# osmocom/osmo-trx

Measured on AMD Instinct MI355X. Metric: Mbursts/s detect+demod (156.25 sym, 4 SPS), higher is better.
Workload: dtype f32

## Files before the change

osmo_trx_amd/csrc/trx_kernel_nb.hip:

```cpp
#include "trx_k4_common.h"
#include "trx_nb_asm.inc"

#define NB_D_LEN    160
#define NB_CZ_LEN   (TRX_CZ_PAD + TRX_CORR_NARROW + TRX_CZ_PAD)
#define NB_SLICE    (K4_XS + NB_D_LEN + NB_CZ_LEN)
#define NB_COMP_ROWS (TRX_DELAY_FILTS + 1)
#define NB_TABLES_FLOATS (TRX_SINCV_LDS + 16 * WAVE + NB_COMP_ROWS * 36 + 16 + 8 * 8 + 5 * WAVE + 5 * WAVE + 2 * 8 * 16)
#define NB_TABLES_BYTES (NB_TABLES_FLOATS * 4)
#define NB_WPB 16
#define NB_POOL_RING 64
#define NB_POOL_UNSET (-1)
#define NB_POOL_END (-2)
#define NB_NO_BURST 0xffffffffu
#define NB_LDS_TAIL (16 + 4 * NB_POOL_RING)
#define NB_LDS_BYTES (NB_TABLES_BYTES + NB_WPB * NB_SLICE * 8 + NB_LDS_TAIL)
#define NB_MAX_TOA 32



typedef float v3f __attribute__((ext_vector_type(3)));
typedef int v4i __attribute__((ext_vector_type(4)));

template <typename T>
__device__ __forceinline__ unsigned lds_addr(const T *p)
// ... 42 lines not shown
		wa4f[((u >> 2) * WAVE + l) * 4 + (u & 3)] = (q < TRX_SINCV_LEN) ? tab->sincv[q] : 0.0f;
	}
	for (int i = threadIdx.x; i < NB_COMP_ROWS * 36; i += blockDim.x) {
		const int f = i / 36, j = i % 36;
		comp[i] = (j >= TRX_FUSED_SH) ? tab->comp_filt[f][j - TRX_FUSED_SH] : 0.0f;
	}
	if (threadIdx.x < 16)
		gdec[threadIdx.x] = tab->dec_taps[threadIdx.x];
	if (threadIdx.x < 128)
		lseq[threadIdx.x] = make_float2(tab->seq[TRX_SEQ_TSC0 + (threadIdx.x >> 4)].taps[threadIdx.x & 15].re,
						tab->seq[TRX_SEQ_TSC0 + (threadIdx.x >> 4)].taps[threadIdx.x & 15].im);
	if (threadIdx.x < 64)
		lhdr[threadIdx.x] = reinterpret_cast<const float *>(&tab->seq[TRX_SEQ_TSC0 + (threadIdx.x >> 3)].gain)[threadIdx.x & 7];
	if (threadIdx.x < WAVE) {
		const PeakConst pc0 = peak_const(threadIdx.x);
		pkcl[0 * WAVE + threadIdx.x] = pc0.flA;
		pkcl[1 * WAVE + threadIdx.x] = pc0.loA;
		pkcl[2 * WAVE + threadIdx.x] = pc0.hiA;
		pkcl[3 * WAVE + threadIdx.x] = pc0.offB;
		pkcl[4 * WAVE + threadIdx.x] = pc0.ratio_off;
		lcn[0 * WAVE + threadIdx.x] = pc0.ratio_off * 8;
		lcn[1 * WAVE + threadIdx.x] = (pc0.flA - 8) * 8;
		lcn[2 * WAVE + threadIdx.x] = pc0.offB;
		const int l = threadIdx.x, e = (-l) & 3;
		const bool sp = l >= 52 && l < 60;
		lcn[3 * WAVE + l] = 8 * (sp ? (l < 56 ? e : e - 2) : (l < 48 ? 4 + 3 * l : 148));
		lcn[4 * WAVE + l] = sp ? (e + (l >= 56 ? 4 : 0)) * K4_NTP * 4 : -1;
	}
	for (int i = lane0; i < NB_SLICE; i += WAVE)
		wbase[i] = make_float2(0.0f, 0.0f);
	if (threadIdx.x == 0) {
		wg_next[0] = NB_WPB;
		wg_next[1] = 0;
	}
	if (threadIdx.x < NB_POOL_RING)
		pool_g[threadIdx.x] = NB_POOL_UNSET;
	__syncthreads();

	const float fs_db = 6.02059991f * __log2f(full_scale);
	const float thr2 = thresh * thresh;
	const float gc0 = thr2 * 1.0001e-5f;
	int t5pk = 0;
	bool t5_ok = true;
	for (int t = 0; t < 8; t++) {
		const int v = (int)(lhdr[8 * t + 5] * 512.0f);
		t5_ok = t5_ok && v >= -8 && v <= 7 && (float)v == lhdr[8 * t + 5] * 512.0f;
		t5pk |= (v & 15) << (4 * t);
	}
	t5pk = uni(t5pk);
	const unsigned long long e8_addr = reinterpret_cast<unsigned long long>(&tab->edge8[0][0][0]);
// ... 161 lines not shown
			float ar = x0.x * ct0, ai = x0.y * ct0;
			ar = fmaf(x1.x, ct1, ar); ai = fmaf(x1.y, ct1, ai);
			ar = fmaf(x2.x, ct2, ar); ai = fmaf(x2.y, ct2, ai);
			const float sr = row_sum(ar), si = row_sum(ai);
			if (lt == 0 && lact)
				dec[li] = cmul(make_float2(sr, si), scale);
		}
		if (hi_tab) {
			const int s0 = 4 * hi_i - 24 - w + lt;
			const c32 *pp = P + ((s0 & 3) * PH_A + PH_M0 + (s0 >> 2));
			const c32 x0 = lds_c32(pp), x1 = lds_c32(pp + 4), x2 = lds_c32(pp + 8);
			float ar = x0.x * ch0, ai = x0.y * ch0;
			ar = fmaf(x1.x, ch1, ar); ai = fmaf(x1.y, ch1, ai);
			ar = fmaf(x2.x, ch2, ar); ai = fmaf(x2.y, ch2, ai);
			const float sr = row_sum(ar), si = row_sum(ai);
			if (lt == 0 && hact && hi_i < 156)
				dec[hi_i] = cmul(make_float2(sr, si), scale);
		}
		wave_sync();
		auto pick = [&](int i) {
			const float d = reinterpret_cast<const float *>(dec + i)[i & 1];
			return __builtin_amdgcn_fmed3f(fmaf((i & 2) ? -0.5f : 0.5f, d, 0.5f), 0.0f, 1.0f);
		};
		const int i0 = (lane < 48) ? 4 + 3 * lane : ((-lane) & 3);
		o.x = pick(i0);
		o.y = pick(lane < 48 ? i0 + 1 : 0);
		o.z = pick(lane < 48 ? i0 + 2 : 0);
		wave_sync();
		return true;
	};

	DIAG_DECL;
	unsigned j_next = 0, b_next = NB_NO_BURST;
	for (unsigned b = b_first; b != NB_NO_BURST; b = b_next) {
		int lane;
		asm volatile("v_mbcnt_lo_u32_b32 %0, -1, 0\n\tv_mbcnt_hi_u32_b32 %0, -1, %0" : "=v"(lane));
		const int ticket = claim_issue(wg_next);
		const unsigned prm0 = (unsigned)uni((int)pre_prm);
		const unsigned max_toa = prm0 >> 16;
		const int tsc = (prm0 >> 8) & 0xff;
		bool leave = ((prm0 & 0xf8ffu) != (unsigned)TRXHIP_TSC) || (max_toa > NB_MAX_TOA) || !t5_ok;

		c32 *const pload = P + (lane & 3) * PH_A + PH_M0 + (lane >> 2);
		float amax = 0.0f, epart = 0.0f;
#ifdef TRX_DIAG
		DIAG_MARK(12);
		asm volatile("s_waitcnt vmcnt(0)" ::: "memory");
		DIAG_MARK(13);
#endif
		if (!leave) {
#pragma unroll
			for (int r = 0; r < NLD; r++) {
				const int i = r * WAVE + lane;
				if (r < NLD - 1 || i < 625) {
					const c32 v = make_float2((float)(int16_t)(pre_i[r] & 0xffffu), (float)(int16_t)(pre_i[r] >> 16));
					pload[16 * r] = v;
					asm("v_max3_f32 %0, %0, |%1|, |%2|" : "+v"(amax) : "v"(v.x), "v"(v.y));
					if (r < 5)
						epart = fmaf(v.x, v.x, fmaf(v.y, v.y, epart));
				}
			}
		} else {
#pragma unroll
			for (int r = 0; r < NLD; r++)
				asm volatile("" :: "v"(pre_i[r]));
		}
		DIAG_MARK(14);
		if (pend_any) {
			float *const so = soft + (size_t)pend_b * 148;
			int *const rp = reinterpret_cast<int *>(results + pend_b);
			const float oe = o.x;
			asm volatile("s_bfm_b64 exec, 48, 0\n\t"
				     "global_store_dwordx3 %0, %1, %2 offset:16\n\t"
				     "s_bfm_b64 exec, 4, 52\n\t"
				     "global_store_dword %3, %4, %2\n\t"
				     "s_mov_b64 exec, %8\n\t"
				     "global_store_dword %5, %6, %7\n\t"
				     "s_mov_b64 exec, -1\n\t"
				     "s_nop 0"
				     :: "v"(lane * 12), "v"(o), "s"(so), "v"(((-lane) & 3) * 4), "v"(oe), "v"(lane * 4), "v"(recw), "s"(rp),
				        "s"(pend_rec ? 0xffull : 0ull)
				     : "memory");
		}
		pend_any = false;
		DIAG_MARK(16);
		j_next = (unsigned)(leave ? claim_take(ticket) : claim_take_behind<5>(ticket));
		b_next = burst_of(j_next);
		if (pooled && (j_next & 15u) == 0u && j_next + 16u >= items)
			pool_draw(j_next, b_next == NB_NO_BURST && j_next >= items, lane);
		DIAG_MARK(17);
		if (b_next != NB_NO_BURST)
			prefetch(b_next, lane);
		DIAG_MARK(15);

		int clip = 0;
		if (!leave) {
			clip = __ballot(amax > TRX_CLIP_THRESH) != 0ull;

			const int len = 16 + (int)max_toa;
			__builtin_assume(len >= 16 && len <= 16 + NB_MAX_TOA);
			const unsigned vd_addr = lds_addr(D) + 8u * (unsigned)lane, vcz_addr = lds_addr(cz) + 8u * (unsigned)lane;
			unsigned long long bad;
			float dr, di;
// ... 127 lines not shown
			}
		}
		if (leave) {
			if (lane == 0) {
				reinterpret_cast<uint8_t *>(redo + TRX_REDO_HDR)[b] = 1;
				if (!left_any)
					__hip_atomic_store(redo, 1u, __ATOMIC_RELAXED, __HIP_MEMORY_SCOPE_AGENT);
			}
			left_any = true;
			continue;
		}
		pend_b = b;
		pend_any = true;
		if (q_n == WAVE)
			flush_records(lane);
		DIAG_MARK(11);
	}
	if (pend_any) {
		int lane;
		asm volatile("v_mbcnt_lo_u32_b32 %0, -1, 0\n\tv_mbcnt_hi_u32_b32 %0, -1, %0" : "=v"(lane));
		float *const so = soft + (size_t)pend_b * 148;
		int *const rp = reinterpret_cast<int *>(results + pend_b);
		const float oe = o.x;
		asm volatile("s_bfm_b64 exec, 48, 0\n\t"
			     "global_store_dwordx3 %0, %1, %2 offset:16\n\t"
			     "s_bfm_b64 exec, 4, 52\n\t"
			     "global_store_dword %3, %4, %2\n\t"
			     "s_mov_b64 exec, %8\n\t"
			     "global_store_dword %5, %6, %7\n\t"
			     "s_mov_b64 exec, -1\n\t"
			     "s_nop 0"
			     :: "v"(lane * 12), "v"(o), "s"(so), "v"(((-lane) & 3) * 4), "v"(oe), "v"(lane * 4), "v"(recw), "s"(rp),
			        "s"(pend_rec ? 0xffull : 0ull)
			     : "memory");
	}
	{
		int lane;
		asm volatile("v_mbcnt_lo_u32_b32 %0, -1, 0\n\tv_mbcnt_hi_u32_b32 %0, -1, %0" : "=v"(lane));
		flush_records(lane);
	}
	DIAG_FLUSH();
	if (pooled) {
		__syncthreads();
		int tid0;
		asm volatile("v_mbcnt_lo_u32_b32 %0, -1, 0\n\tv_mbcnt_hi_u32_b32 %0, -1, %0" : "=v"(tid0));
		if (tid0 == 0 && atomicAdd(wg_next + 1, 1) == 0) {
			const unsigned d = __hip_atomic_fetch_add(pool_ctr + 1, 1u, __ATOMIC_ACQ_REL, __HIP_MEMORY_SCOPE_AGENT);
			if (d == gridDim.x - 1u) {
				__hip_atomic_store(pool_ctr, 0u, __ATOMIC_RELAXED, __HIP_MEMORY_SCOPE_AGENT);
				__hip_atomic_store(pool_ctr + 1, 0u, __ATOMIC_RELEASE, __HIP_MEMORY_SCOPE_AGENT);
			}
		}
	}
}
```

osmo_trx_amd/csrc/trx_nb_asm.inc:

```
#define NB_ASM_GDEC_OFF 29968
#define NB_ASM_LSEQ_OFF 32848
#define NB_ASM_DEC_MAX_NACT 60
#define NB_ASM_CORR_LANE0 19
#define NB_ASM_CORR_MAX_LEN 45
#define NB_ASM_CLOBBERS "v64", "v65", "v66", "v67", "v68", "v69", "v70", "v71", "v72", "v73", "v74", "v75", "v76", "v77", "v78", "v79", "v80", "v81", "v82", "v83", "v84", "v85", "v86", "v87", "v88", "v89", "v90", "v91", "v92", "v93", "v94", "v95", "v96", "v97", "v98", "v99", "v100", "v101", "v102", "v103", "v104", "v105", "v106", "v107", "v108", "v109", "v110", "v111", "v112", "v113", "v114", "v115", "v116", "v117", "v118", "v119", "v120", "v121", "v122", "v123", "v124", "v125", "v126", "v127", "s87", "s88", "s89", "s90", "s91", "s92", "s93", "s94", "s95", "s96", "s97", "s98", "s99", "vcc", "scc", "memory"
#define NB_ASM_DEC \
	"s_cmp_gt_u32 %[nact], 60\n\t" \
	"s_cbranch_scc1 .Lnb_dec_wide\n\t" \
	"s_sub_u32 s88, 60, %[nact]\n\t" \
	"s_lshr_b64 exec, -1, s88\n\t" \
	"ds_read_b128 v[120:123], %[zero] offset:29968\n\t" \
	"ds_read_b128 v[124:127], %[zero] offset:29984\n\t" \
	"ds_read_b64 v[98:99], %[pd] offset:1440\n\t" \
	"ds_read_b64 v[100:101], %[pd] offset:2880\n\t" \
	"ds_read_b64 v[102:103], %[pd] offset:4320\n\t" \
	"ds_read_b64 v[96:97], %[pd] offset:0\n\t" \
	"s_waitcnt lgkmcnt(3)\n\t" \
	"v_pk_mul_f32 v[64:65], v[98:99], v[120:121] op_sel:[0,0] op_sel_hi:[1,0]\n\t" \
	"s_waitcnt lgkmcnt(2)\n\t" \
	"v_pk_mul_f32 v[66:67], v[100:101], v[120:121] op_sel:[0,1] op_sel_hi:[1,1]\n\t" \
	"s_waitcnt lgkmcnt(1)\n\t" \
	"v_pk_mul_f32 v[68:69], v[102:103], v[122:123] op_sel:[0,0] op_sel_hi:[1,0]\n\t" \
	"v_pk_add_f32 v[104:105], v[64:65], v[66:67]\n\t" \
	"s_waitcnt lgkmcnt(0)\n\t" \
// ... 1448 lines not shown
	"s_add_u32 s95, s95, %[cb]\n\t" \
	"v_readlane_b32 %[ssum], v81, 0\n\t" \
	"s_mov_b64 exec, -1\n\t" \
	"s_sub_u32 s96, 0, s88\n\t" \
	"s_cmp_gt_u32 s96, 36\n\t" \
	"s_cbranch_scc1 .Lnb_tl_wait_end\n\t" \
	"s_mov_b32 %[ok], 1\n\t" \
	"v_add_u32_e32 v112, s94, %[kic]\n\t" \
	"s_add_u32 s96, s92, 1\n\t" \
	"s_lshr_b32 s96, s96, 2\n\t" \
	"s_mul_i32 s96, s96, -5752\n\t" \
	"s_add_u32 s96, s96, 1440\n\t" \
	"v_add_u32_e32 v113, s96, v112\n\t" \
	"s_add_u32 s96, s92, 2\n\t" \
	"s_lshr_b32 s96, s96, 2\n\t" \
	"s_mul_i32 s96, s96, -5752\n\t" \
	"s_add_u32 s96, s96, 2880\n\t" \
	"v_add_u32_e32 v114, s96, v112\n\t" \
	"s_add_u32 s96, s92, 3\n\t" \
	"s_lshr_b32 s96, s96, 2\n\t" \
	"s_mul_i32 s96, s96, -5752\n\t" \
	"s_add_u32 s96, s96, 4320\n\t" \
	"v_add_u32_e32 v115, s96, v112\n\t" \
	"s_mov_b32 exec_hi, 0x0ff0ffff\n\t" \
	"ds_read_b64 v[72:73], v112 offset:96\n\t" \
	"ds_read_b64 v[74:75], v113 offset:96\n\t" \
	"ds_read_b64 v[76:77], v114 offset:96\n\t" \
	"ds_read_b64 v[78:79], v115 offset:96\n\t" \
	"ds_read_b64 v[80:81], v112 offset:104\n\t" \
	"ds_read_b64 v[82:83], v113 offset:104\n\t" \
	"ds_read_b64 v[84:85], v114 offset:104\n\t" \
	"ds_read_b64 v[86:87], v115 offset:104\n\t" \
	"ds_read_b64 v[88:89], v112 offset:112\n\t" \
	"ds_read_b64 v[90:91], v113 offset:112\n\t" \
	"ds_read_b64 v[92:93], v114 offset:112\n\t" \
	"ds_read_b64 v[94:95], v115 offset:112\n\t" \
	"v_add_u32_e32 v116, %[db], %[l16]\n\t" \
	"v_cmp_lt_i32_e32 vcc, -1, %[ktp]\n\t" \
	"v_add_u32_e32 v117, %[db], %[ktp]\n\t" \
	"v_mov_b32_e32 v118, s95\n\t" \
	"v_mov_b64_e32 v[64:65], 0\n\t" \
	"v_mov_b64_e32 v[66:67], 0\n\t" \
	"v_mov_b64_e32 v[68:69], 0\n\t" \
	"v_cndmask_b32_e32 v117, v118, v117, vcc\n\t" \
	"s_waitcnt vmcnt(0)\n\t" \
	"ds_write_b128 v116, v[120:123]\n\t" \
	"ds_read_b128 v[104:107], v117\n\t" \
	"ds_read_b128 v[108:111], v117 offset:16\n\t" \
	"ds_read_b64 v[96:97], v112 offset:120\n\t" \
	"ds_read_b64 v[98:99], v113 offset:120\n\t" \
	"ds_read_b64 v[100:101], v114 offset:120\n\t" \
	"ds_read_b64 v[102:103], v115 offset:120\n\t" \
	"s_waitcnt lgkmcnt(5)\n\t" \
	"v_pk_fma_f32 v[64:65], v[72:73], v[104:105], v[64:65] op_sel:[0,0,0] op_sel_hi:[1,0,1]\n\t" \
	"v_pk_fma_f32 v[66:67], v[80:81], v[104:105], v[66:67] op_sel:[0,0,0] op_sel_hi:[1,0,1]\n\t" \
	"v_pk_fma_f32 v[68:69], v[88:89], v[104:105], v[68:69] op_sel:[0,0,0] op_sel_hi:[1,0,1]\n\t" \
	"v_pk_fma_f32 v[64:65], v[74:75], v[104:105], v[64:65] op_sel:[0,1,0] op_sel_hi:[1,1,1]\n\t" \
	"v_pk_fma_f32 v[66:67], v[82:83], v[104:105], v[66:67] op_sel:[0,1,0] op_sel_hi:[1,1,1]\n\t" \
	"v_pk_fma_f32 v[68:69], v[90:91], v[104:105], v[68:69] op_sel:[0,1,0] op_sel_hi:[1,1,1]\n\t" \
	"v_pk_fma_f32 v[64:65], v[76:77], v[106:107], v[64:65] op_sel:[0,0,0] op_sel_hi:[1,0,1]\n\t" \
	"v_pk_fma_f32 v[66:67], v[84:85], v[106:107], v[66:67] op_sel:[0,0,0] op_sel_hi:[1,0,1]\n\t" \
	"v_pk_fma_f32 v[68:69], v[92:93], v[106:107], v[68:69] op_sel:[0,0,0] op_sel_hi:[1,0,1]\n\t" \
	"v_pk_fma_f32 v[64:65], v[78:79], v[106:107], v[64:65] op_sel:[0,1,0] op_sel_hi:[1,1,1]\n\t" \
	"v_pk_fma_f32 v[66:67], v[86:87], v[106:107], v[66:67] op_sel:[0,1,0] op_sel_hi:[1,1,1]\n\t" \
	"v_pk_fma_f32 v[68:69], v[94:95], v[106:107], v[68:69] op_sel:[0,1,0] op_sel_hi:[1,1,1]\n\t" \
	"ds_read_b128 v[104:107], v117 offset:32\n\t" \
	"ds_read_b64 v[72:73], v112 offset:128\n\t" \
	"ds_read_b64 v[74:75], v113 offset:128\n\t" \
	"ds_read_b64 v[76:77], v114 offset:128\n\t" \
	"ds_read_b64 v[78:79], v115 offset:128\n\t" \
	"s_waitcnt lgkmcnt(5)\n\t" \
	"v_pk_fma_f32 v[64:65], v[80:81], v[108:109], v[64:65] op_sel:[0,0,0] op_sel_hi:[1,0,1]\n\t" \
	"v_pk_fma_f32 v[66:67], v[88:89], v[108:109], v[66:67] op_sel:[0,0,0] op_sel_hi:[1,0,1]\n\t" \
	"v_pk_fma_f32 v[68:69], v[96:97], v[108:109], v[68:69] op_sel:[0,0,0] op_sel_hi:[1,0,1]\n\t" \
	"v_pk_fma_f32 v[64:65], v[82:83], v[108:109], v[64:65] op_sel:[0,1,0] op_sel_hi:[1,1,1]\n\t" \
	"v_pk_fma_f32 v[66:67], v[90:91], v[108:109], v[66:67] op_sel:[0,1,0] op_sel_hi:[1,1,1]\n\t" \
	"v_pk_fma_f32 v[68:69], v[98:99], v[108:109], v[68:69] op_sel:[0,1,0] op_sel_hi:[1,1,1]\n\t" \
	"v_pk_fma_f32 v[64:65], v[84:85], v[110:111], v[64:65] op_sel:[0,0,0] op_sel_hi:[1,0,1]\n\t" \
	"v_pk_fma_f32 v[66:67], v[92:93], v[110:111], v[66:67] op_sel:[0,0,0] op_sel_hi:[1,0,1]\n\t" \
	"v_pk_fma_f32 v[68:69], v[100:101], v[110:111], v[68:69] op_sel:[0,0,0] op_sel_hi:[1,0,1]\n\t" \
	"v_pk_fma_f32 v[64:65], v[86:87], v[110:111], v[64:65] op_sel:[0,1,0] op_sel_hi:[1,1,1]\n\t" \
	"v_pk_fma_f32 v[66:67], v[94:95], v[110:111], v[66:67] op_sel:[0,1,0] op_sel_hi:[1,1,1]\n\t" \
	"v_pk_fma_f32 v[68:69], v[102:103], v[110:111], v[68:69] op_sel:[0,1,0] op_sel_hi:[1,1,1]\n\t" \
	"ds_read_b128 v[108:111], v117 offset:48\n\t" \
	"ds_read_b64 v[80:81], v112 offset:136\n\t" \
	"ds_read_b64 v[82:83], v113 offset:136\n\t" \
	"ds_read_b64 v[84:85], v114 offset:136\n\t" \
	"ds_read_b64 v[86:87], v115 offset:136\n\t" \
	"s_waitcnt lgkmcnt(5)\n\t" \
	"v_pk_fma_f32 v[64:65], v[88:89], v[104:105], v[64:65] op_sel:[0,0,0] op_sel_hi:[1,0,1]\n\t" \
	"v_pk_fma_f32 v[66:67], v[96:97], v[104:105], v[66:67] op_sel:[0,0,0] op_sel_hi:[1,0,1]\n\t" \
	"v_pk_fma_f32 v[68:69], v[72:73], v[104:105], v[68:69] op_sel:[0,0,0] op_sel_hi:[1,0,1]\n\t" \
	"v_pk_fma_f32 v[64:65], v[90:91], v[104:105], v[64:65] op_sel:[0,1,0] op_sel_hi:[1,1,1]\n\t" \
	"v_pk_fma_f32 v[66:67], v[98:99], v[104:105], v[66:67] op_sel:[0,1,0] op_sel_hi:[1,1,1]\n\t" \
	"v_pk_fma_f32 v[68:69], v[74:75], v[104:105], v[68:69] op_sel:[0,1,0] op_sel_hi:[1,1,1]\n\t" \
	"v_pk_fma_f32 v[64:65], v[92:93], v[106:107], v[64:65] op_sel:[0,0,0] op_sel_hi:[1,0,1]\n\t" \
	"v_pk_fma_f32 v[66:67], v[100:101], v[106:107], v[66:67] op_sel:[0,0,0] op_sel_hi:[1,0,1]\n\t" \
	"v_pk_fma_f32 v[68:69], v[76:77], v[106:107], v[68:69] op_sel:[0,0,0] op_sel_hi:[1,0,1]\n\t" \
	"v_pk_fma_f32 v[64:65], v[94:95], v[106:107], v[64:65] op_sel:[0,1,0] op_sel_hi:[1,1,1]\n\t" \
	"v_pk_fma_f32 v[66:67], v[102:103], v[106:107], v[66:67] op_sel:[0,1,0] op_sel_hi:[1,1,1]\n\t" \
	"v_pk_fma_f32 v[68:69], v[78:79], v[106:107], v[68:69] op_sel:[0,1,0] op_sel_hi:[1,1,1]\n\t" \
	"ds_read_b128 v[104:107], v117 offset:64\n\t" \
	"ds_read_b64 v[88:89], v112 offset:144\n\t" \
	"ds_read_b64 v[90:91], v113 offset:144\n\t" \
	"ds_read_b64 v[92:93], v114 offset:144\n\t" \
	"ds_read_b64 v[94:95], v115 offset:144\n\t" \
	"s_waitcnt lgkmcnt(5)\n\t" \
	"v_pk_fma_f32 v[64:65], v[96:97], v[108:109], v[64:65] op_sel:[0,0,0] op_sel_hi:[1,0,1]\n\t" \
	"v_pk_fma_f32 v[66:67], v[72:73], v[108:109], v[66:67] op_sel:[0,0,0] op_sel_hi:[1,0,1]\n\t" \
	"v_pk_fma_f32 v[68:69], v[80:81], v[108:109], v[68:69] op_sel:[0,0,0] op_sel_hi:[1,0,1]\n\t" \
	"v_pk_fma_f32 v[64:65], v[98:99], v[108:109], v[64:65] op_sel:[0,1,0] op_sel_hi:[1,1,1]\n\t" \
	"v_pk_fma_f32 v[66:67], v[74:75], v[108:109], v[66:67] op_sel:[0,1,0] op_sel_hi:[1,1,1]\n\t" \
	"v_pk_fma_f32 v[68:69], v[82:83], v[108:109], v[68:69] op_sel:[0,1,0] op_sel_hi:[1,1,1]\n\t" \
	"v_pk_fma_f32 v[64:65], v[100:101], v[110:111], v[64:65] op_sel:[0,0,0] op_sel_hi:[1,0,1]\n\t" \
	"v_pk_fma_f32 v[66:67], v[76:77], v[110:111], v[66:67] op_sel:[0,0,0] op_sel_hi:[1,0,1]\n\t" \
	"v_pk_fma_f32 v[68:69], v[84:85], v[110:111], v[68:69] op_sel:[0,0,0] op_sel_hi:[1,0,1]\n\t" \
	"v_pk_fma_f32 v[64:65], v[102:103], v[110:111], v[64:65] op_sel:[0,1,0] op_sel_hi:[1,1,1]\n\t" \
	"v_pk_fma_f32 v[66:67], v[78:79], v[110:111], v[66:67] op_sel:[0,1,0] op_sel_hi:[1,1,1]\n\t" \
	"v_pk_fma_f32 v[68:69], v[86:87], v[110:111], v[68:69] op_sel:[0,1,0] op_sel_hi:[1,1,1]\n\t" \
	"ds_read_b128 v[108:111], v117 offset:80\n\t" \
	"ds_read_b64 v[96:97], v112 offset:152\n\t" \
	"ds_read_b64 v[98:99], v113 offset:152\n\t" \
	"ds_read_b64 v[100:101], v114 offset:152\n\t" \
	"ds_read_b64 v[102:103], v115 offset:152\n\t" \
	"s_waitcnt lgkmcnt(5)\n\t" \
	"v_pk_fma_f32 v[64:65], v[72:73], v[104:105], v[64:65] op_sel:[0,0,0] op_sel_hi:[1,0,1]\n\t" \
	"v_pk_fma_f32 v[66:67], v[80:81], v[104:105], v[66:67] op_sel:[0,0,0] op_sel_hi:[1,0,1]\n\t" \
	"v_pk_fma_f32 v[68:69], v[88:89], v[104:105], v[68:69] op_sel:[0,0,0] op_sel_hi:[1,0,1]\n\t" \
	"v_pk_fma_f32 v[64:65], v[74:75], v[104:105], v[64:65] op_sel:[0,1,0] op_sel_hi:[1,1,1]\n\t" \
	"v_pk_fma_f32 v[66:67], v[82:83], v[104:105], v[66:67] op_sel:[0,1,0] op_sel_hi:[1,1,1]\n\t" \
	"v_pk_fma_f32 v[68:69], v[90:91], v[104:105], v[68:69] op_sel:[0,1,0] op_sel_hi:[1,1,1]\n\t" \
	"v_pk_fma_f32 v[64:65], v[76:77], v[106:107], v[64:65] op_sel:[0,0,0] op_sel_hi:[1,0,1]\n\t" \
	"v_pk_fma_f32 v[66:67], v[84:85], v[106:107], v[66:67] op_sel:[0,0,0] op_sel_hi:[1,0,1]\n\t" \
	"v_pk_fma_f32 v[68:69], v[92:93], v[106:107], v[68:69] op_sel:[0,0,0] op_sel_hi:[1,0,1]\n\t" \
	"v_pk_fma_f32 v[64:65], v[78:79], v[106:107], v[64:65] op_sel:[0,1,0] op_sel_hi:[1,1,1]\n\t" \
	"v_pk_fma_f32 v[66:67], v[86:87], v[106:107], v[66:67] op_sel:[0,1,0] op_sel_hi:[1,1,1]\n\t" \
	"v_pk_fma_f32 v[68:69], v[94:95], v[106:107], v[68:69] op_sel:[0,1,0] op_sel_hi:[1,1,1]\n\t" \
	"s_waitcnt lgkmcnt(0)\n\t" \
	"v_pk_fma_f32 v[64:65], v[80:81], v[108:109], v[64:65] op_sel:[0,0,0] op_sel_hi:[1,0,1]\n\t" \
	"v_pk_fma_f32 v[66:67], v[88:89], v[108:109], v[66:67] op_sel:[0,0,0] op_sel_hi:[1,0,1]\n\t" \
	"v_pk_fma_f32 v[68:69], v[96:97], v[108:109], v[68:69] op_sel:[0,0,0] op_sel_hi:[1,0,1]\n\t" \
	"v_pk_fma_f32 v[64:65], v[82:83], v[108:109], v[64:65] op_sel:[0,1,0] op_sel_hi:[1,1,1]\n\t" \
	"v_pk_fma_f32 v[66:67], v[90:91], v[108:109], v[66:67] op_sel:[0,1,0] op_sel_hi:[1,1,1]\n\t" \
	"v_pk_fma_f32 v[68:69], v[98:99], v[108:109], v[68:69] op_sel:[0,1,0] op_sel_hi:[1,1,1]\n\t" \
	"v_pk_fma_f32 v[64:65], v[84:85], v[110:111], v[64:65] op_sel:[0,0,0] op_sel_hi:[1,0,1]\n\t" \
	"v_pk_fma_f32 v[66:67], v[92:93], v[110:111], v[66:67] op_sel:[0,0,0] op_sel_hi:[1,0,1]\n\t" \
	"v_pk_fma_f32 v[68:69], v[100:101], v[110:111], v[68:69] op_sel:[0,0,0] op_sel_hi:[1,0,1]\n\t" \
	"v_pk_fma_f32 v[64:65], v[86:87], v[110:111], v[64:65] op_sel:[0,1,0] op_sel_hi:[1,1,1]\n\t" \
	"v_pk_fma_f32 v[66:67], v[94:95], v[110:111], v[66:67] op_sel:[0,1,0] op_sel_hi:[1,1,1]\n\t" \
	"v_pk_fma_f32 v[68:69], v[102:103], v[110:111], v[68:69] op_sel:[0,1,0] op_sel_hi:[1,1,1]\n\t" \
	"s_nop 0\n\t" \
	"v_add_f32_dpp v64, v64, v64 row_shl:4 row_mask:0x8 bank_mask:0xf\n\t" \
	"v_add_f32_dpp v65, v65, v65 row_shl:4 row_mask:0x8 bank_mask:0xf\n\t" \
	"v_mul_f32_dpp %[d1], v119, v66 quad_perm:[1,0,3,2] row_mask:0xf bank_mask:0xf\n\t" \
	"v_mul_f32_dpp %[d2], v119, v68 quad_perm:[2,1,0,3] row_mask:0xf bank_mask:0xf\n\t" \
	"v_mul_f32_dpp %[d0], v119, v64 quad_perm:[0,3,2,1] row_mask:0xf bank_mask:0xf\n\t" \
	"v_fmac_f32_dpp %[d1], v119, v67 quad_perm:[0,3,2,1] row_mask:0xf bank_mask:0xf\n\t" \
	"v_fmac_f32_dpp %[d2], v119, v69 quad_perm:[1,0,3,2] row_mask:0xf bank_mask:0xf\n\t" \
	"v_fmac_f32_dpp %[d0], v119, v65 quad_perm:[3,2,1,0] row_mask:0xf bank_mask:0xf\n\t" \
	"s_mov_b64 exec, -1\n\t" \
	"s_branch .Lnb_tl_end\n\t" \
	".Lnb_tl_wait_end:\n\t" \
	"s_waitcnt vmcnt(0)\n\t" \
	".Lnb_tl_end:\n\t"
#define NB_ASM_FIRG \
	"s_ashr_i32 s88, %[nk], 7\n\t" \
	"s_and_b32 s89, %[nk], 127\n\t" \
	"s_lshr_b32 s90, s89, 1\n\t" \
	"s_cmp_ge_u32 s89, 2\n\t" \
	"s_cselect_b32 s90, s90, 64\n\t" \
	"s_sub_u32 s91, -18, s88\n\t" \
	"s_and_b32 s92, s91, 3\n\t" \
	"s_ashr_i32 s93, s91, 2\n\t" \
	"s_mul_i32 s94, s92, 180\n\t" \
	"s_add_u32 s94, s94, s93\n\t" \
	"s_lshl3_add_u32 s94, s94, %[pb]\n\t" \
	"s_mul_i32 s95, s90, 144\n\t" \
	"s_add_u32 s95, s95, %[cb]\n\t" \
	"v_add_u32_e32 v112, s94, %[kic]\n\t" \
	"s_add_u32 s96, s92, 1\n\t" \
	"s_lshr_b32 s96, s96, 2\n\t" \
	"s_mul_i32 s96, s96, -5752\n\t" \
	"s_add_u32 s96, s96, 1440\n\t" \
// ... 160 lines not shown
```

Before: 1053.

## Reuse sample registers across taps via wave_shr accumulator rotation in demod tail

Rewrites the tail demodulation FIR in the NB inline assembly. Instead of reloading sliding sample windows from LDS each step, it keeps the sample registers fixed and rotates the partial-sum accumulators across lanes with DPP wave_shr, then loads all coefficient blocks up front. This drops the per-step sample ds_read_b64 traffic and the staggered waits. The lane-to-symbol mapping changes as a result, so the output pick indices, special-lane tables and store exec masks and offsets are updated to match. The cost is extra DPP moves, exec mask switching and a more fragile lane mapping.

New measurement: 1069 (median of 6 runs). +1.6%, better.

```diff
diff --git a/osmo_trx_amd/csrc/trx_kernel_nb.hip b/osmo_trx_amd/csrc/trx_kernel_nb.hip
--- a/osmo_trx_amd/csrc/trx_kernel_nb.hip
+++ b/osmo_trx_amd/csrc/trx_kernel_nb.hip
@@ -88,10 +88,10 @@
 		lcn[0 * WAVE + threadIdx.x] = pc0.ratio_off * 8;
 		lcn[1 * WAVE + threadIdx.x] = (pc0.flA - 8) * 8;
 		lcn[2 * WAVE + threadIdx.x] = pc0.offB;
-		const int l = threadIdx.x, e = (-l) & 3;
-		const bool sp = l >= 52 && l < 60;
-		lcn[3 * WAVE + l] = 8 * (sp ? (l < 56 ? e : e - 2) : (l < 48 ? 4 + 3 * l : 148));
-		lcn[4 * WAVE + l] = sp ? (e + (l >= 56 ? 4 : 0)) * K4_NTP * 4 : -1;
+		const int l = threadIdx.x, e = (l - 52) / 3, t = (l - 52) % 3;
+		const bool sp = l >= 52;
+		lcn[3 * WAVE + l] = 8 * (sp ? (t == 0 ? e : t == 1 ? e + 3 : e - 3) : 4 + 3 * (l < 49 ? l : 49));
+		lcn[4 * WAVE + l] = sp ? (e + (t == 2 ? 4 : 0)) * K4_NTP * 4 : -1;
 	}
 	for (int i = lane0; i < NB_SLICE; i += WAVE)
 		wbase[i] = make_float2(0.0f, 0.0f);
@@ -299,10 +299,11 @@
 			const float d = reinterpret_cast<const float *>(dec + i)[i & 1];
 			return __builtin_amdgcn_fmed3f(fmaf((i & 2) ? -0.5f : 0.5f, d, 0.5f), 0.0f, 1.0f);
 		};
-		const int i0 = (lane < 48) ? 4 + 3 * lane : ((-lane) & 3);
+		const bool reg = lane >= 2 && lane < 50;
+		const int i0 = reg ? 3 * lane - 2 : ((((lane - 54) * 11) >> 5) & 3);
 		o.x = pick(i0);
-		o.y = pick(lane < 48 ? i0 + 1 : 0);
-		o.z = pick(lane < 48 ? i0 + 2 : 0);
+		o.y = pick(reg ? i0 + 1 : 0);
+		o.z = pick(reg ? i0 + 2 : 0);
 		wave_sync();
 		return true;
 	};
@@ -347,15 +348,16 @@
 			float *const so = soft + (size_t)pend_b * 148;
 			int *const rp = reinterpret_cast<int *>(results + pend_b);
 			const float oe = o.x;
-			asm volatile("s_bfm_b64 exec, 48, 0\n\t"
+			asm volatile("s_bfm_b64 exec, 48, 2\n\t"
 				     "global_store_dwordx3 %0, %1, %2 offset:16\n\t"
-				     "s_bfm_b64 exec, 4, 52\n\t"
+				     "s_mov_b32 exec_lo, 0\n\t"
+			     "s_mov_b32 exec_hi, 0x92400000\n\t"
 				     "global_store_dword %3, %4, %2\n\t"
 				     "s_mov_b64 exec, %8\n\t"
 				     "global_store_dword %5, %6, %7\n\t"
 				     "s_mov_b64 exec, -1\n\t"
 				     "s_nop 0"
-				     :: "v"(lane * 12), "v"(o), "s"(so), "v"(((-lane) & 3) * 4), "v"(oe), "v"(lane * 4), "v"(recw), "s"(rp),
+				     :: "v"((lane - 2) * 12), "v"(o), "s"(so), "v"((((lane - 54) * 11) >> 5) * 4), "v"(oe), "v"(lane * 4), "v"(recw), "s"(rp),
 				        "s"(pend_rec ? 0xffull : 0ull)
 				     : "memory");
 		}
@@ -529,15 +531,16 @@
 		float *const so = soft + (size_t)pend_b * 148;
 		int *const rp = reinterpret_cast<int *>(results + pend_b);
 		const float oe = o.x;
-		asm volatile("s_bfm_b64 exec, 48, 0\n\t"
+		asm volatile("s_bfm_b64 exec, 48, 2\n\t"
 			     "global_store_dwordx3 %0, %1, %2 offset:16\n\t"
-			     "s_bfm_b64 exec, 4, 52\n\t"
+		     "s_mov_b32 exec_lo, 0\n\t"
+		     "s_mov_b32 exec_hi, 0x92400000\n\t"
 			     "global_store_dword %3, %4, %2\n\t"
 			     "s_mov_b64 exec, %8\n\t"
 			     "global_store_dword %5, %6, %7\n\t"
 			     "s_mov_b64 exec, -1\n\t"
 			     "s_nop 0"
-			     :: "v"(lane * 12), "v"(o), "s"(so), "v"(((-lane) & 3) * 4), "v"(oe), "v"(lane * 4), "v"(recw), "s"(rp),
+			     :: "v"((lane - 2) * 12), "v"(o), "s"(so), "v"((((lane - 54) * 11) >> 5) * 4), "v"(oe), "v"(lane * 4), "v"(recw), "s"(rp),
 			        "s"(pend_rec ? 0xffull : 0ull)
 			     : "memory");
 	}
diff --git a/osmo_trx_amd/csrc/trx_nb_asm.inc b/osmo_trx_amd/csrc/trx_nb_asm.inc
--- a/osmo_trx_amd/csrc/trx_nb_asm.inc
+++ b/osmo_trx_amd/csrc/trx_nb_asm.inc
@@ -1494,7 +1494,6 @@
 	"s_mul_i32 s96, s96, -5752\n\t" \
 	"s_add_u32 s96, s96, 4320\n\t" \
 	"v_add_u32_e32 v115, s96, v112\n\t" \
-	"s_mov_b32 exec_hi, 0x0ff0ffff\n\t" \
 	"ds_read_b64 v[72:73], v112 offset:96\n\t" \
 	"ds_read_b64 v[74:75], v113 offset:96\n\t" \
 	"ds_read_b64 v[76:77], v114 offset:96\n\t" \
@@ -1517,120 +1516,116 @@
 	"v_cndmask_b32_e32 v117, v118, v117, vcc\n\t" \
 	"s_waitcnt vmcnt(0)\n\t" \
 	"ds_write_b128 v116, v[120:123]\n\t" \
-	"ds_read_b128 v[104:107], v117\n\t" \
-	"ds_read_b128 v[108:111], v117 offset:16\n\t" \
-	"ds_read_b64 v[96:97], v112 offset:120\n\t" \
-	"ds_read_b64 v[98:99], v113 offset:120\n\t" \
-	"ds_read_b64 v[100:101], v114 offset:120\n\t" \
-	"ds_read_b64 v[102:103], v115 offset:120\n\t" \
-	"s_waitcnt lgkmcnt(5)\n\t" \
-	"v_pk_fma_f32 v[64:65], v[72:73], v[104:105], v[64:65] op_sel:[0,0,0] op_sel_hi:[1,0,1]\n\t" \
-	"v_pk_fma_f32 v[66:67], v[80:81], v[104:105], v[66:67] op_sel:[0,0,0] op_sel_hi:[1,0,1]\n\t" \
-	"v_pk_fma_f32 v[68:69], v[88:89], v[104:105], v[68:69] op_sel:[0,0,0] op_sel_hi:[1,0,1]\n\t" \
-	"v_pk_fma_f32 v[64:65], v[74:75], v[104:105], v[64:65] op_sel:[0,1,0] op_sel_hi:[1,1,1]\n\t" \
-	"v_pk_fma_f32 v[66:67], v[82:83], v[104:105], v[66:67] op_sel:[0,1,0] op_sel_hi:[1,1,1]\n\t" \
-	"v_pk_fma_f32 v[68:69], v[90:91], v[104:105], v[68:69] op_sel:[0,1,0] op_sel_hi:[1,1,1]\n\t" \
-	"v_pk_fma_f32 v[64:65], v[76:77], v[106:107], v[64:65] op_sel:[0,0,0] op_sel_hi:[1,0,1]\n\t" \
-	"v_pk_fma_f32 v[66:67], v[84:85], v[106:107], v[66:67] op_sel:[0,0,0] op_sel_hi:[1,0,1]\n\t" \
-	"v_pk_fma_f32 v[68:69], v[92:93], v[106:107], v[68:69] op_sel:[0,0,0] op_sel_hi:[1,0,1]\n\t" \
-	"v_pk_fma_f32 v[64:65], v[78:79], v[106:107], v[64:65] op_sel:[0,1,0] op_sel_hi:[1,1,1]\n\t" \
-	"v_pk_fma_f32 v[66:67], v[86:87], v[106:107], v[66:67] op_sel:[0,1,0] op_sel_hi:[1,1,1]\n\t" \
-	"v_pk_fma_f32 v[68:69], v[94:95], v[106:107], v[68:69] op_sel:[0,1,0] op_sel_hi:[1,1,1]\n\t" \
+	"ds_read_b128 v[96:99], v117 offset:0\n\t" \
+	"ds_read_b128 v[100:103], v117 offset:16\n\t" \
 	"ds_read_b128 v[104:107], v117 offset:32\n\t" \
-	"ds_read_b64 v[72:73], v112 offset:128\n\t" \
-	"ds_read_b64 v[74:75], v113 offset:128\n\t" \
-	"ds_read_b64 v[76:77], v114 offset:128\n\t" \
-	"ds_read_b64 v[78:79], v115 offset:128\n\t" \
-	"s_waitcnt lgkmcnt(5)\n\t" \
-	"v_pk_fma_f32 v[64:65], v[80:81], v[108:109], v[64:65] op_sel:[0,0,0] op_sel_hi:[1,0,1]\n\t" \
-	"v_pk_fma_f32 v[66:67], v[88:89], v[108:109], v[66:67] op_sel:[0,0,0] op_sel_hi:[1,0,1]\n\t" \
-	"v_pk_fma_f32 v[68:69], v[96:97], v[108:109], v[68:69] op_sel:[0,0,0] op_sel_hi:[1,0,1]\n\t" \
-	"v_pk_fma_f32 v[64:65], v[82:83], v[108:109], v[64:65] op_sel:[0,1,0] op_sel_hi:[1,1,1]\n\t" \
-	"v_pk_fma_f32 v[66:67], v[90:91], v[108:109], v[66:67] op_sel:[0,1,0] op_sel_hi:[1,1,1]\n\t" \
-	"v_pk_fma_f32 v[68:69], v[98:99], v[108:109], v[68:69] op_sel:[0,1,0] op_sel_hi:[1,1,1]\n\t" \
-	"v_pk_fma_f32 v[64:65], v[84:85], v[110:111], v[64:65] op_sel:[0,0,0] op_sel_hi:[1,0,1]\n\t" \
-	"v_pk_fma_f32 v[66:67], v[92:93], v[110:111], v[66:67] op_sel:[0,0,0] op_sel_hi:[1,0,1]\n\t" \
-	"v_pk_fma_f32 v[68:69], v[100:101], v[110:111], v[68:69] op_sel:[0,0,0] op_sel_hi:[1,0,1]\n\t" \
-	"v_pk_fma_f32 v[64:65], v[86:87], v[110:111], v[64:65] op_sel:[0,1,0] op_sel_hi:[1,1,1]\n\t" \
-	"v_pk_fma_f32 v[66:67], v[94:95], v[110:111], v[66:67] op_sel:[0,1,0] op_sel_hi:[1,1,1]\n\t" \
-	"v_pk_fma_f32 v[68:69], v[102:103], v[110:111], v[68:69] op_sel:[0,1,0] op_sel_hi:[1,1,1]\n\t" \
 	"ds_read_b128 v[108:111], v117 offset:48\n\t" \
-	"ds_read_b64 v[80:81], v112 offset:136\n\t" \
-	"ds_read_b64 v[82:83], v113 offset:136\n\t" \
-	"ds_read_b64 v[84:85], v114 offset:136\n\t" \
-	"ds_read_b64 v[86:87], v115 offset:136\n\t" \
-	"s_waitcnt lgkmcnt(5)\n\t" \
+	"ds_read_b128 v[124:127], v117 offset:64\n\t" \
+	"s_waitcnt lgkmcnt(4)\n\t" \
+	"ds_read_b128 v[120:123], v117 offset:80\n\t" \
+	"v_pk_fma_f32 v[64:65], v[72:73], v[96:97], v[64:65] op_sel:[0,0,0] op_sel_hi:[1,0,1]\n\t" \
+	"v_pk_fma_f32 v[66:67], v[80:81], v[96:97], v[66:67] op_sel:[0,0,0] op_sel_hi:[1,0,1]\n\t" \
+	"v_pk_fma_f32 v[68:69], v[88:89], v[96:97], v[68:69] op_sel:[0,0,0] op_sel_hi:[1,0,1]\n\t" \
+	"v_pk_fma_f32 v[64:65], v[74:75], v[96:97], v[64:65] op_sel:[0,1,0] op_sel_hi:[1,1,1]\n\t" \
+	"v_pk_fma_f32 v[66:67], v[82:83], v[96:97], v[66:67] op_sel:[0,1,0] op_sel_hi:[1,1,1]\n\t" \
+	"v_pk_fma_f32 v[68:69], v[90:91], v[96:97], v[68:69] op_sel:[0,1,0] op_sel_hi:[1,1,1]\n\t" \
+	"v_pk_fma_f32 v[64:65], v[76:77], v[98:99], v[64:65] op_sel:[0,0,0] op_sel_hi:[1,0,1]\n\t" \
+	"v_pk_fma_f32 v[66:67], v[84:85], v[98:99], v[66:67] op_sel:[0,0,0] op_sel_hi:[1,0,1]\n\t" \
+	"v_pk_fma_f32 v[68:69], v[92:93], v[98:99], v[68:69] op_sel:[0,0,0] op_sel_hi:[1,0,1]\n\t" \
+	"v_pk_fma_f32 v[64:65], v[78:79], v[98:99], v[64:65] op_sel:[0,1,0] op_sel_hi:[1,1,1]\n\t" \
+	"v_pk_fma_f32 v[66:67], v[86:87], v[98:99], v[66:67] op_sel:[0,1,0] op_sel_hi:[1,1,1]\n\t" \
+	"v_pk_fma_f32 v[68:69], v[94:95], v[98:99], v[68:69] op_sel:[0,1,0] op_sel_hi:[1,1,1]\n\t" \
+	"s_waitcnt lgkmcnt(4)\n\t" \
+	"v_pk_fma_f32 v[64:65], v[80:81], v[100:101], v[64:65] op_sel:[0,0,0] op_sel_hi:[1,0,1]\n\t" \
+	"v_pk_fma_f32 v[66:67], v[88:89], v[100:101], v[66:67] op_sel:[0,0,0] op_sel_hi:[1,0,1]\n\t" \
+	"v_mov_b32_dpp v68, v68 wave_shr:1 row_mask:0xf bank_mask:0xf bound_ctrl:0\n\t" \
+	"v_mov_b32_dpp v69, v69 wave_shr:1 row_mask:0xf bank_mask:0xf bound_ctrl:0\n\t" \
+	"v_pk_fma_f32 v[64:65], v[82:83], v[100:101], v[64:65] op_sel:[0,1,0] op_sel_hi:[1,1,1]\n\t" \
+	"v_pk_fma_f32 v[66:67], v[90:91], v[100:101], v[66:67] op_sel:[0,1,0] op_sel_hi:[1,1,1]\n\t" \
+	"v_pk_fma_f32 v[68:69], v[72:73], v[100:101], v[68:69] op_sel:[0,0,0] op_sel_hi:[1,0,1]\n\t" \
+	"v_pk_fma_f32 v[64:65], v[84:85], v[102:103], v[64:65] op_sel:[0,0,0] op_sel_hi:[1,0,1]\n\t" \
+	"v_pk_fma_f32 v[66:67], v[92:93], v[102:103], v[66:67] op_sel:[0,0,0] op_sel_hi:[1,0,1]\n\t" \
+	"v_pk_fma_f32 v[68:69], v[74:75], v[100:101], v[68:69] op_sel:[0,1,0] op_sel_hi:[1,1,1]\n\t" \
+	"v_pk_fma_f32 v[64:65], v[86:87], v[102:103], v[64:65] op_sel:[0,1,0] op_sel_hi:[1,1,1]\n\t" \
+	"v_pk_fma_f32 v[66:67], v[94:95], v[102:103], v[66:67] op_sel:[0,1,0] op_sel_hi:[1,1,1]\n\t" \
+	"v_pk_fma_f32 v[68:69], v[76:77], v[102:103], v[68:69] op_sel:[0,0,0] op_sel_hi:[1,0,1]\n\t" \
+	"s_waitcnt lgkmcnt(3)\n\t" \
 	"v_pk_fma_f32 v[64:65], v[88:89], v[104:105], v[64:65] op_sel:[0,0,0] op_sel_hi:[1,0,1]\n\t" \
-	"v_pk_fma_f32 v[66:67], v[96:97], v[104:105], v[66:67] op_sel:[0,0,0] op_sel_hi:[1,0,1]\n\t" \
-	"v_pk_fma_f32 v[68:69], v[72:73], v[104:105], v[68:69] op_sel:[0,0,0] op_sel_hi:[1,0,1]\n\t" \
+	"s_bfm_b64 exec, 52, 0\n\t" \
+	"v_mov_b32_dpp v66, v66 wave_shr:1 row_mask:0xf bank_mask:0xf bound_ctrl:0\n\t" \
+	"v_mov_b32_dpp v67, v67 wave_shr:1 row_mask:0xf bank_mask:0xf bound_ctrl:0\n\t" \
+	"s_mov_b64 exec, -1\n\t" \
+	"v_pk_fma_f32 v[68:69], v[78:79], v[102:103], v[68:69] op_sel:[0,1,0] op_sel_hi:[1,1,1]\n\t" \
 	"v_pk_fma_f32 v[64:65], v[90:91], v[104:105], v[64:65] op_sel:[0,1,0] op_sel_hi:[1,1,1]\n\t" \
-	"v_pk_fma_f32 v[66:67], v[98:99], v[104:105], v[66:67] op_sel:[0,1,0] op_sel_hi:[1,1,1]\n\t" \
-	"v_pk_fma_f32 v[68:69], v[74:75], v[104:105], v[68:69] op_sel:[0,1,0] op_sel_hi:[1,1,1]\n\t" \
+	"v_pk_fma_f32 v[66:67], v[72:73], v[104:105], v[66:67] op_sel:[0,0,0] op_sel_hi:[1,0,1]\n\t" \
+	"v_pk_fma_f32 v[68:69], v[80:81], v[104:105], v[68:69] op_sel:[0,0,0] op_sel_hi:[1,0,1]\n\t" \
 	"v_pk_fma_f32 v[64:65], v[92:93], v[106:107], v[64:65] op_sel:[0,0,0] op_sel_hi:[1,0,1]\n\t" \
-	"v_pk_fma_f32 v[66:67], v[100:101], v[106:107], v[66:67] op_sel:[0,0,0] op_sel_hi:[1,0,1]\n\t" \
-	"v_pk_fma_f32 v[68:69], v[76:77], v[106:107], v[68:69] op_sel:[0,0,0] op_sel_hi:[1,0,1]\n\t" \
+	"v_pk_fma_f32 v[66:67], v[74:75], v[104:105], v[66:67] op_sel:[0,1,0] op_sel_hi:[1,1,1]\n\t" \
+	"v_pk_fma_f32 v[68:69], v[82:83], v[104:105], v[68:69] op_sel:[0,1,0] op_sel_hi:[1,1,1]\n\t" \
 	"v_pk_fma_f32 v[64:65], v[94:95], v[106:107], v[64:65] op_sel:[0,1,0] op_sel_hi:[1,1,1]\n\t" \
-	"v_pk_fma_f32 v[66:67], v[102:103], v[106:107], v[66:67] op_sel:[0,1,0] op_sel_hi:[1,1,1]\n\t" \
-	"v_pk_fma_f32 v[68:69], v[78:79], v[106:107], v[68:69] op_sel:[0,1,0] op_sel_hi:[1,1,1]\n\t" \
-	"ds_read_b128 v[104:107], v117 offset:64\n\t" \
-	"ds_read_b64 v[88:89], v112 offset:144\n\t" \
-	"ds_read_b64 v[90:91], v113 offset:144\n\t" \
-	"ds_read_b64 v[92:93], v114 offset:144\n\t" \
-	"ds_read_b64 v[94:95], v115 offset:144\n\t" \
-	"s_waitcnt lgkmcnt(5)\n\t" \
-	"v_pk_fma_f32 v[64:65], v[96:97], v[108:109], v[64:65] op_sel:[0,0,0] op_sel_hi:[1,0,1]\n\t" \
-	"v_pk_fma_f32 v[66:67], v[72:73], v[108:109], v[66:67] op_sel:[0,0,0] op_sel_hi:[1,0,1]\n\t" \
-	"v_pk_fma_f32 v[68:69], v[80:81], v[108:109], v[68:69] op_sel:[0,0,0] op_sel_hi:[1,0,1]\n\t" \
-	"v_pk_fma_f32 v[64:65], v[98:99], v[108:109], v[64:65] op_sel:[0,1,0] op_sel_hi:[1,1,1]\n\t" \
-	"v_pk_fma_f32 v[66:67], v[74:75], v[108:109], v[66:67] op_sel:[0,1,0] op_sel_hi:[1,1,1]\n\t" \
-	"v_pk_fma_f32 v[68:69], v[82:83], v[108:109], v[68:69] op_sel:[0,1,0] op_sel_hi:[1,1,1]\n\t" \
-	"v_pk_fma_f32 v[64:65], v[100:101], v[110:111], v[64:65] op_sel:[0,0,0] op_sel_hi:[1,0,1]\n\t" \
-	"v_pk_fma_f32 v[66:67], v[76:77], v[110:111], v[66:67] op_sel:[0,0,0] op_sel_hi:[1,0,1]\n\t" \
-	"v_pk_fma_f32 v[68:69], v[84:85], v[110:111], v[68:69] op_sel:[0,0,0] op_sel_hi:[1,0,1]\n\t" \
-	"v_pk_fma_f32 v[64:65], v[102:103], v[110:111], v[64:65] op_sel:[0,1,0] op_sel_hi:[1,1,1]\n\t" \
-	"v_pk_fma_f32 v[66:67], v[78:79], v[110:111], v[66:67] op_sel:[0,1,0] op_sel_hi:[1,1,1]\n\t" \
-	"v_pk_fma_f32 v[68:69], v[86:87], v[110:111], v[68:69] op_sel:[0,1,0] op_sel_hi:[1,1,1]\n\t" \
-	"ds_read_b128 v[108:111], v117 offset:80\n\t" \
-	"ds_read_b64 v[96:97], v112 offset:152\n\t" \
-	"ds_read_b64 v[98:99], v113 offset:152\n\t" \
-	"ds_read_b64 v[100:101], v114 offset:152\n\t" \
-	"ds_read_b64 v[102:103], v115 offset:152\n\t" \
-	"s_waitcnt lgkmcnt(5)\n\t" \
-	"v_pk_fma_f32 v[64:65], v[72:73], v[104:105], v[64:65] op_sel:[0,0,0] op_sel_hi:[1,0,1]\n\t" \
-	"v_pk_fma_f32 v[66:67], v[80:81], v[104:105], v[66:67] op_sel:[0,0,0] op_sel_hi:[1,0,1]\n\t" \
-	"v_pk_fma_f32 v[68:69], v[88:89], v[104:105], v[68:69] op_sel:[0,0,0] op_sel_hi:[1,0,1]\n\t" \
-	"v_pk_fma_f32 v[64:65], v[74:75], v[104:105], v[64:65] op_sel:[0,1,0] op_sel_hi:[1,1,1]\n\t" \
-	"v_pk_fma_f32 v[66:67], v[82:83], v[104:105], v[66:67] op_sel:[0,1,0] op_sel_hi:[1,1,1]\n\t" \
-	"v_pk_fma_f32 v[68:69], v[90:91], v[104:105], v[68:69] op_sel:[0,1,0] op_sel_hi:[1,1,1]\n\t" \
-	"v_pk_fma_f32 v[64:65], v[76:77], v[106:107], v[64:65] op_sel:[0,0,0] op_sel_hi:[1,0,1]\n\t" \
-	"v_pk_fma_f32 v[66:67], v[84:85], v[106:107], v[66:67] op_sel:[0,0,0] op_sel_hi:[1,0,1]\n\t" \
-	"v_pk_fma_f32 v[68:69], v[92:93], v[106:107], v[68:69] op_sel:[0,0,0] op_sel_hi:[1,0,1]\n\t" \
-	"v_pk_fma_f32 v[64:65], v[78:79], v[106:107], v[64:65] op_sel:[0,1,0] op_sel_hi:[1,1,1]\n\t" \
-	"v_pk_fma_f32 v[66:67], v[86:87], v[106:107], v[66:67] op_sel:[0,1,0] op_sel_hi:[1,1,1]\n\t" \
-	"v_pk_fma_f32 v[68:69], v[94:95], v[106:107], v[68:69] op_sel:[0,1,0] op_sel_hi:[1,1,1]\n\t" \
-	"s_waitcnt lgkmcnt(0)\n\t" \
-	"v_pk_fma_f32 v[64:65], v[80:81], v[108:109], v[64:65] op_sel:[0,0,0] op_sel_hi:[1,0,1]\n\t" \
-	"v_pk_fma_f32 v[66:67], v[88:89], v[108:109], v[66:67] op_sel:[0,0,0] op_sel_hi:[1,0,1]\n\t" \
-	"v_pk_fma_f32 v[68:69], v[96:97], v[108:109], v[68:69] op_sel:[0,0,0] op_sel_hi:[1,0,1]\n\t" \
-	"v_pk_fma_f32 v[64:65], v[82:83], v[108:109], v[64:65] op_sel:[0,1,0] op_sel_hi:[1,1,1]\n\t" \
-	"v_pk_fma_f32 v[66:67], v[90:91], v[108:109], v[66:67] op_sel:[0,1,0] op_sel_hi:[1,1,1]\n\t" \
-	"v_pk_fma_f32 v[68:69], v[98:99], v[108:109], v[68:69] op_sel:[0,1,0] op_sel_hi:[1,1,1]\n\t" \
-	"v_pk_fma_f32 v[64:65], v[84:85], v[110:111], v[64:65] op_sel:[0,0,0] op_sel_hi:[1,0,1]\n\t" \
-	"v_pk_fma_f32 v[66:67], v[92:93], v[110:111], v[66:67] op_sel:[0,0,0] op_sel_hi:[1,0,1]\n\t" \
-	"v_pk_fma_f32 v[68:69], v[100:101], v[110:111], v[68:69] op_sel:[0,0,0] op_sel_hi:[1,0,1]\n\t" \
-	"v_pk_fma_f32 v[64:65], v[86:87], v[110:111], v[64:65] op_sel:[0,1,0] op_sel_hi:[1,1,1]\n\t" \
-	"v_pk_fma_f32 v[66:67], v[94:95], v[110:111], v[66:67] op_sel:[0,1,0] op_sel_hi:[1,1,1]\n\t" \
-	"v_pk_fma_f32 v[68:69], v[102:103], v[110:111], v[68:69] op_sel:[0,1,0] op_sel_hi:[1,1,1]\n\t" \
-	"s_nop 0\n\t" \
-	"v_add_f32_dpp v64, v64, v64 row_shl:4 row_mask:0x8 bank_mask:0xf\n\t" \
-	"v_add_f32_dpp v65, v65, v65 row_shl:4 row_mask:0x8 bank_mask:0xf\n\t" \
-	"v_mul_f32_dpp %[d1], v119, v66 quad_perm:[1,0,3,2] row_mask:0xf bank_mask:0xf\n\t" \
-	"v_mul_f32_dpp %[d2], v119, v68 quad_perm:[2,1,0,3] row_mask:0xf bank_mask:0xf\n\t" \
-	"v_mul_f32_dpp %[d0], v119, v64 quad_perm:[0,3,2,1] row_mask:0xf bank_mask:0xf\n\t" \
-	"v_fmac_f32_dpp %[d1], v119, v67 quad_perm:[0,3,2,1] row_mask:0xf bank_mask:0xf\n\t" \
-	"v_fmac_f32_dpp %[d2], v119, v69 quad_perm:[1,0,3,2] row_mask:0xf bank_mask:0xf\n\t" \
-	"v_fmac_f32_dpp %[d0], v119, v65 quad_perm:[3,2,1,0] row_mask:0xf bank_mask:0xf\n\t" \
+	"v_pk_fma_f32 v[66:67], v[76:77], v[106:107], v[66:67] op_sel:[0,0,0] op_sel_hi:[1,0,1]\n\t" \
+	"v_pk_fma_f32 v[68:69], v[84:85], v[106:107], v[68:69] op_sel:[0,0,0] op_sel_hi:[1,0,1]\n\t" \
+	"v_mov_b32_dpp v64, v64 wave_shr:1 row_mask:0xf bank_mask:0xf bound_ctrl:0\n\t" \
+	"v_mov_b32_dpp v65, v65 wave_shr:1 row_mask:0xf bank_mask:0xf bound_ctrl:0\n\t" \
+	"v_pk_fma_f32 v[66:67], v[78:79], v[106:107], v[66:67] op_sel:[0,1,0] op_sel_hi:[1,1,1]\n\t" \
+	"v_pk_fma_f32 v[68:69], v[86:87], v[106:107], v[68:69] op_sel:[0,1,0] op_sel_hi:[1,1,1]\n\t" \
+	"s_waitcnt lgkmcnt(2)\n\t" \
+	"v_pk_fma_f32 v[64:65], v[72:73], v[108:109], v[64:65] op_sel:[0,0,0] op_sel_hi:[1,0,1]\n\t" \
+	"v_pk_fma_f32 v[66:67], v[80:81], v[108:109], v[66:67] op_sel:[0,0,0] op_sel_hi:[1,0,1]\n\t" \
+	"v_pk_fma_f32 v[68:69], v[88:89], v[108:109], v[68:69] op_sel:[0,0,0] op_sel_hi:[1,0,1]\n\t" \
+	"v_pk_fma_f32 v[64:65], v[74:75], v[108:109], v[64:65] op_sel:[0,1,0] op_sel_hi:[1,1,1]\n\t" \
+	"v_pk_fma_f32 v[66:67], v[82:83], v[108:109], v[66:67] op_sel:[0,1,0] op_sel_hi:[1,1,1]\n\t" \
+	"v_pk_fma_f32 v[68:69], v[90:91], v[108:109], v[68:69] op_sel:[0,1,0] op_sel_hi:[1,1,1]\n\t" \
+	"v_pk_fma_f32 v[64:65], v[76:77], v[110:111], v[64:65] op_sel:[0,0,0] op_sel_hi:[1,0,1]\n\t" \
+	"v_pk_fma_f32 v[66:67], v[84:85], v[110:111], v[66:67] op_sel:[0,0,0] op_sel_hi:[1,0,1]\n\t" \
+	"v_pk_fma_f32 v[68:69], v[92:93], v[110:111], v[68:69] op_sel:[0,0,0] op_sel_hi:[1,0,1]\n\t" \
+	"v_pk_fma_f32 v[64:65], v[78:79], v[110:111], v[64:65] op_sel:[0,1,0] op_sel_hi:[1,1,1]\n\t" \
+	"v_pk_fma_f32 v[66:67], v[86:87], v[110:111], v[66:67] op_sel:[0,1,0] op_sel_hi:[1,1,1]\n\t" \
+	"v_pk_fma_f32 v[68:69], v[94:95], v[110:111], v[68:69] op_sel:[0,1,0] op_sel_hi:[1,1,1]\n\t" \
+	"s_waitcnt lgkmcnt(1)\n\t" \
+	"v_pk_fma_f32 v[64:65], v[80:81], v[124:125], v[64:65] op_sel:[0,0,0] op_sel_hi:[1,0,1]\n\t" \
+	"v_pk_fma_f32 v[66:67], v[88:89], v[124:125], v[66:67] op_sel:[0,0,0] op_sel_hi:[1,0,1]\n\t" \
+	"v_mov_b32_dpp v68, v68 wave_shr:1 row_mask:0xf bank_mask:0xf bound_ctrl:0\n\t" \
+	"v_mov_b32_dpp v69, v69 wave_shr:1 row_mask:0xf bank_mask:0xf bound_ctrl:0\n\t" \
+	"v_pk_fma_f32 v[64:65], v[82:83], v[124:125], v[64:65] op_sel:[0,1,0] op_sel_hi:[1,1,1]\n\t" \
+	"v_pk_fma_f32 v[66:67], v[90:91], v[124:125], v[66:67] op_sel:[0,1,0] op_sel_hi:[1,1,1]\n\t" \
+	"v_pk_fma_f32 v[68:69], v[72:73], v[124:125], v[68:69] op_sel:[0,0,0] op_sel_hi:[1,0,1]\n\t" \
+	"v_pk_fma_f32 v[64:65], v[84:85], v[126:127], v[64:65] op_sel:[0,0,0] op_sel_hi:[1,0,1]\n\t" \
+	"v_pk_fma_f32 v[66:67], v[92:93], v[126:127], v[66:67] op_sel:[0,0,0] op_sel_hi:[1,0,1]\n\t" \
+	"v_pk_fma_f32 v[68:69], v[74:75], v[124:125], v[68:69] op_sel:[0,1,0] op_sel_hi:[1,1,1]\n\t" \
+	"v_pk_fma_f32 v[64:65], v[86:87], v[126:127], v[64:65] op_sel:[0,1,0] op_sel_hi:[1,1,1]\n\t" \
+	"v_pk_fma_f32 v[66:67], v[94:95], v[126:127], v[66:67] op_sel:[0,1,0] op_sel_hi:[1,1,1]\n\t" \
+	"v_pk_fma_f32 v[68:69], v[76:77], v[126:127], v[68:69] op_sel:[0,0,0] op_sel_hi:[1,0,1]\n\t" \
+	"s_waitcnt lgkmcnt(0)\n\t" \
+	"v_pk_fma_f32 v[64:65], v[88:89], v[120:121], v[64:65] op_sel:[0,0,0] op_sel_hi:[1,0,1]\n\t" \
+	"s_bfm_b64 exec, 52, 0\n\t" \
+	"v_mov_b32_dpp v66, v66 wave_shr:1 row_mask:0xf bank_mask:0xf bound_ctrl:0\n\t" \
+	"v_mov_b32_dpp v67, v67 wave_shr:1 row_mask:0xf bank_mask:0xf bound_ctrl:0\n\t" \
 	"s_mov_b64 exec, -1\n\t" \
+	"v_pk_fma_f32 v[68:69], v[78:79], v[126:127], v[68:69] op_sel:[0,1,0] op_sel_hi:[1,1,1]\n\t" \
+	"v_pk_fma_f32 v[64:65], v[90:91], v[120:121], v[64:65] op_sel:[0,1,0] op_sel_hi:[1,1,1]\n\t" \
+	"v_pk_fma_f32 v[66:67], v[72:73], v[120:121], v[66:67] op_sel:[0,0,0] op_sel_hi:[1,0,1]\n\t" \
+	"v_pk_fma_f32 v[68:69], v[80:81], v[120:121], v[68:69] op_sel:[0,0,0] op_sel_hi:[1,0,1]\n\t" \
+	"v_pk_fma_f32 v[64:65], v[92:93], v[122:123], v[64:65] op_sel:[0,0,0] op_sel_hi:[1,0,1]\n\t" \
+	"v_pk_fma_f32 v[66:67], v[74:75], v[120:121], v[66:67] op_sel:[0,1,0] op_sel_hi:[1,1,1]\n\t" \
+	"v_pk_fma_f32 v[68:69], v[82:83], v[120:121], v[68:69] op_sel:[0,1,0] op_sel_hi:[1,1,1]\n\t" \
+	"v_pk_fma_f32 v[64:65], v[94:95], v[122:123], v[64:65] op_sel:[0,1,0] op_sel_hi:[1,1,1]\n\t" \
+	"v_pk_fma_f32 v[66:67], v[76:77], v[122:123], v[66:67] op_sel:[0,0,0] op_sel_hi:[1,0,1]\n\t" \
+	"v_pk_fma_f32 v[68:69], v[84:85], v[122:123], v[68:69] op_sel:[0,0,0] op_sel_hi:[1,0,1]\n\t" \
+	"v_mov_b32_dpp v64, v64 wave_shr:1 row_mask:0xf bank_mask:0xf bound_ctrl:0\n\t" \
+	"v_mov_b32_dpp v65, v65 wave_shr:1 row_mask:0xf bank_mask:0xf bound_ctrl:0\n\t" \
+	"v_pk_fma_f32 v[66:67], v[78:79], v[122:123], v[66:67] op_sel:[0,1,0] op_sel_hi:[1,1,1]\n\t" \
+	"v_pk_fma_f32 v[68:69], v[86:87], v[122:123], v[68:69] op_sel:[0,1,0] op_sel_hi:[1,1,1]\n\t" \
+	"s_mov_b32 exec_lo, 0\n\t" \
+	"s_mov_b32 exec_hi, 0xfff00000\n\t" \
+	"v_pk_add_f32 v[64:65], v[64:65], v[66:67]\n\t" \
+	"s_mov_b64 exec, -1\n\t" \
+	"v_mul_f32_dpp %[d1], v119, v66 quad_perm:[3,2,1,0] row_mask:0xf bank_mask:0xf\n\t" \
+	"v_mul_f32_dpp %[d2], v119, v68 quad_perm:[0,3,2,1] row_mask:0xf bank_mask:0xf\n\t" \
+	"v_mul_f32_dpp %[d0], v119, v64 quad_perm:[2,1,0,3] row_mask:0xf bank_mask:0xf\n\t" \
+	"v_fmac_f32_dpp %[d1], v119, v67 quad_perm:[2,1,0,3] row_mask:0xf bank_mask:0xf\n\t" \
+	"v_fmac_f32_dpp %[d2], v119, v69 quad_perm:[3,2,1,0] row_mask:0xf bank_mask:0xf\n\t" \
+	"v_fmac_f32_dpp %[d0], v119, v65 quad_perm:[1,0,3,2] row_mask:0xf bank_mask:0xf\n\t" \
 	"s_branch .Lnb_tl_end\n\t" \
 	".Lnb_tl_wait_end:\n\t" \
 	"s_waitcnt vmcnt(0)\n\t" \
```
